# Kira7dn/Low_Level_Feature_Extraction

Hardware: AMD Instinct MI355X
Metric: images/sec, 1080p batch, full colors+shapes+shadows pipeline @1/2/4/8 MI355X (higher is better)
Workload: dtype u8

## Files before the change

### low_level_feature_extraction_amd/_build.py

```python
from __future__ import annotations

import os
import shutil
import subprocess
import sys

PKG = os.path.dirname(os.path.abspath(__file__))
ROOT = os.path.dirname(PKG)
CSRC = os.path.join(PKG, "csrc")
LIB = os.path.join(PKG, "libllfe.so")
SOURCES = ["llfe_context.cpp", "llfe_pipeline.cpp", "llfe_stages.cpp", "llfe_resize.cpp", "llfe_decode.cpp", "llfe_colors_images.cpp", "llfe_shapes_images.cpp", "contours.cpp", "png_decode.cpp", "jpeg_decode.cpp", "stencil.hip", "stencil_stream.hip", "hysteresis.hip", "unique.hip", "kmeans.hip", "kmeans_big.hip", "resize.hip", "contours_gpu.hip",
           "cvresize.hip", "text.hip", "gather.hip", "font.hip", "font_bits.hip", "jpeg_huff.hip", "png_inflate.hip", "thumb_images.hip", "jpeg_images.hip"]
HEADERS = ["llfe_ctx.h", "llfe_internal.h", "contours.h", "kmeans_common.h", "jpeg_huff_core.h", "jpeg_desc_check.h", "jpeg_recon_core.h", "jpeg_images.h", "jpeg_orient.h", "png_inflate_core.h", "host_fanout.h"]
RECOMPILE = [("kmeans.hip", "kmeans_wide", ["-DLLFE_KM_WIDE=1", "-DLLFE_KM_THREADS=512", "-DLLFE_KM_UNROLL=4"])]
ARCH = os.environ.get("LLFE_OFFLOAD_ARCH", "gfx950")
ILP_SCHED = set(filter(None, os.environ.get("LLFE_ILP_SCHED", "stencil_stream.hip,kmeans.hip").split(",")))


def _hipcc() -> str:
    for c in (os.environ.get("HIPCC"), "/opt/rocm/bin/hipcc", shutil.which("hipcc")):
        if c and os.path.exists(c):
            return c
    raise RuntimeError("hipcc not found: the llfe HIP backend cannot be built")


def _stale() -> bool:
    if not os.path.exists(LIB):
        return True
    t = os.path.getmtime(LIB)
    deps = [os.path.join(CSRC, f) for f in SOURCES + HEADERS] + [os.path.join(ROOT, "include", "llfe.h"), __file__]
    return any(os.path.getmtime(d) > t for d in deps)


def build(force: bool = False, verbose: bool = False) -> str:
    if not force and not _stale():
        return LIB
    objs = []
    hipcc = _hipcc()
    common = ["-O3", "-fPIC", "-std=c++17", "-ffp-contract=off", f"-I{os.path.join(ROOT, 'include')}",
              "-Wall", "-Wno-unused-function", "-Wno-unused-variable",
              *os.environ.get("LLFE_EXTRA_FLAGS", "").split()]
    tmpdir = os.path.join(PKG, "build")
    os.makedirs(tmpdir, exist_ok=True)
    procs = []
    for src, stem, defs in [(s, s, []) for s in SOURCES] + RECOMPILE:
        obj = os.path.join(tmpdir, stem + ".o" if stem != src else src + ".o")
        objs.append(obj)
        if src in ("contours.cpp", "png_decode.cpp", "jpeg_decode.cpp"):
            lang = ["-x", "c++"]
        else:
            lang = ["-x", "hip", f"--offload-arch={ARCH}"]
        extra = ["-fno-slp-vectorize"] if src == "stencil_stream.hip" else []
        if src in ILP_SCHED:
            extra += ["-mllvm", "-amdgpu-sched-strategy=iterative-ilp"]
        cmd = [hipcc, *common, *lang, *extra, *defs, "-c", os.path.join(CSRC, src), "-o", obj]
        if verbose:
            print(" ".join(cmd), file=sys.stderr)
        procs.append((cmd, subprocess.Popen(cmd, stdout=subprocess.PIPE, stderr=subprocess.STDOUT)))
    failed = []
    for cmd, p in procs:
        out, _ = p.communicate()
        if p.returncode != 0:
            failed.append((cmd, out.decode(errors="replace")))
        elif verbose and out:
            print(out.decode(errors="replace"), file=sys.stderr)
    if failed:
        msg = "\n\n".join(" ".join(c) + "\n" + o for c, o in failed)
        raise RuntimeError("libllfe build failed:\n" + msg)
    tmp = LIB + ".tmp"
    cmd = [hipcc, "-shared", "-fPIC", f"--offload-arch={ARCH}", *objs, "-o", tmp, "-lpthread", "-lz", "-ldl"]
    subprocess.run(cmd, check=True)
    os.replace(tmp, LIB)
    return LIB


if __name__ == "__main__":
    print(build(force="--force" in sys.argv, verbose=True))
```

### low_level_feature_extraction_amd/csrc/kmeans.hip

```cpp
#include "kmeans_common.h"

#include <mutex>
#include <type_traits>

namespace llfe {
namespace {

#ifndef LLFE_KM_CELL_MIN
#define LLFE_KM_CELL_MIN 8192
#endif
constexpr int kCellMinCubes = LLFE_KM_CELL_MIN;
#ifndef LLFE_KM_SPLIT
#define LLFE_KM_SPLIT 0
#endif
#ifndef LLFE_KM_LLOYD_QUEUE
#define LLFE_KM_LLOYD_QUEUE 0
#endif
#ifndef LLFE_KM_SUPS
#define LLFE_KM_SUPS 1
#endif
#ifndef LLFE_KM_WIDE
#define LLFE_KM_WIDE 0
#endif
#ifndef LLFE_KM_THREADS
#define LLFE_KM_THREADS 256
#endif
constexpr int KT = LLFE_KM_THREADS;
constexpr int KW = KT / 64;
constexpr int STEP = 256;
constexpr float kFar = 1e30f;

using km::cvrng_double;
using km::cvrng_next;
using km::splitmix64;

__device__ __forceinline__ float uni(float v) {
    return __int_as_float(__builtin_amdgcn_readfirstlane(__float_as_int(v)));
}

__device__ __forceinline__ float d2(float x, float y, float z, float cx, float cy, float cz) {
    float t0 = x - cx, t1 = y - cy, t2 = z - cz;
    float d = t0 * t0;
    d = __builtin_fmaf(t1, t1, d);
    d = __builtin_fmaf(t2, t2, d);
    return d;
}

struct P3 {
    float x, y, z;
};
__device__ __forceinline__ P3 unpack(uint32_t k) {
    return P3{(float)((k >> 16) & 255u), (float)((k >> 8) & 255u), (float)(k & 255u)};
}

struct Cent {
    float x[kMaxK], y[kMaxK], z[kMaxK];
};

__device__ __forceinline__ int label5(const P3 &p, const Cent &c, float &best) {
    best = d2(p.x, p.y, p.z, c.x[0], c.y[0], c.z[0]);
    int l = 0;
#pragma unroll
    for (int k = 1; k < kMaxK; k++) {
        float d = d2(p.x, p.y, p.z, c.x[k], c.y[k], c.z[k]);
        bool lt = d < best;
        best = lt ? d : best;
        l = lt ? k : l;
    }
    return l;
}

typedef float f2 __attribute__((ext_vector_type(2)));
typedef uint16_t u16x2 __attribute__((ext_vector_type(2)));
struct CentP {
    f2 x[3], y[3], z[3];
};

__device__ __forceinline__ CentP pack_centres(const Cent &c) {
    CentP r;
#pragma unroll
    for (int j = 0; j < 3; j++) {
        const int a = 2 * j, b = 2 * j + 1;
        r.x[j] = f2{c.x[a], b < kMaxK ? c.x[b] : kFar};
        r.y[j] = f2{c.y[a], b < kMaxK ? c.y[b] : kFar};
        r.z[j] = f2{c.z[a], b < kMaxK ? c.z[b] : kFar};
    }
    return r;
}

__device__ __forceinline__ int label5p(uint32_t key, const CentP &c) {
    const float x = (float)((key >> 16) & 255u), y = (float)((key >> 8) & 255u), z = (float)(key & 255u);
    const f2 px = f2{x, x}, py = f2{y, y}, pz = f2{z, z};
    f2 d[3];
#pragma unroll
    for (int j = 0; j < 3; j++) {
        const f2 t0 = px - c.x[j], t1 = py - c.y[j], t2 = pz - c.z[j];
        f2 dd = t0 * t0;
        dd = __builtin_elementwise_fma(t1, t1, dd);
        dd = __builtin_elementwise_fma(t2, t2, dd);
        d[j] = dd;
    }
    const float m = fminf(fminf(fminf(d[0].x, d[0].y), fminf(d[1].x, d[1].y)), d[2].x);
    int l = 4;
    l = d[1].y == m ? 3 : l;
    l = d[1].x == m ? 2 : l;
    l = d[0].y == m ? 1 : l;
    l = d[0].x == m ? 0 : l;
    return l;
}

constexpr int PF = 4;
constexpr int kSelSteps = ((4 * 256 * 256 + 3 + STEP - 1) / STEP + KW - 1) / KW + 1;
constexpr int SEL_U = 4;
#ifndef LLFE_KM_UNROLL
#define LLFE_KM_UNROLL 2
#endif
#ifndef LLFE_KM_SPLIT_MIN
#define LLFE_KM_SPLIT_MIN 1
#endif
constexpr bool kSplitOn = LLFE_KM_SPLIT_MIN <= 64;
constexpr int kPend = 128;
constexpr int kPendIdxBits = 18;
#ifndef LLFE_KM_PP_SPLIT_MIN
#define LLFE_KM_PP_SPLIT_MIN 8
#endif
constexpr int kPPSplitMin = LLFE_KM_PP_SPLIT_MIN;
#ifndef LLFE_KM_PPRUN
#define LLFE_KM_PPRUN 4
#endif
constexpr int kPPRun = LLFE_KM_PPRUN;
constexpr int ring_size(int need) { return need <= 256 ? 256 : (need <= 512 ? 512 : 1024); }
constexpr int kStage = ring_size(127 + 64 * LLFE_KM_UNROLL);
static_assert(kStage >= 127 + 64 * LLFE_KM_UNROLL && (kStage & (kStage - 1)) == 0, "boundary-colour ring too small");

__device__ __forceinline__ uint4 load_step(const uint32_t *pts, int s, int se_full, int lane) {
    if (s < se_full) return *(const uint4 *)(pts + (size_t)s * STEP + lane * 4);
    return make_uint4(0u, 0u, 0u, 0u);
}

template <typename T>
__device__ __forceinline__ T wave_sum(T v) {
#pragma unroll
    for (int off = 32; off > 0; off >>= 1) v += __shfl_xor(v, off);
    return v;
}

struct KmSmem {
    unsigned long long accA[kMaxK][KT];
    unsigned long long accB[kMaxK][KT];
    union {
        unsigned long long red[32][20];
        int cs[KW][256];
    };
    unsigned long long wtot[KW][3];
    unsigned long long scan_w[KW];
    double dred[KW];
    double maxd[KW];
    int maxi[KW];
    float c[kMaxK][3];
    float cprev[kMaxK][3];
    float cc[kMaxK][3];
    long long sums[kMaxK][3];
    int counts[kMaxK];
    int moved_idx[kMaxK];
    int moved_lbl[kMaxK];
    int n_moved;
    int found_step[3];
    unsigned long long found_excl[3];
    int ci[3];
    int flag;
    int task;
    int next_chunk;
    unsigned long long fail_pts;
    unsigned long long split_cubes, split_pts;
    uint32_t split_walks, split_partial;
    union {
        struct {
            unsigned long long psum[3][kParts];
            unsigned long long pD[kParts];
            unsigned long long wchunk[3][KW];
            int marg[kMaxK * kMaxK + 6 * kMaxK];
            int margc[kMaxK * kMaxK + 6 * kMaxK];
            int margs[kMaxK * kMaxK + 6 * kMaxK];
        } ppw;
        uint32_t pend[KW][kPend];
    };
    unsigned long long pex[3];
    unsigned long long S[3];
    uint32_t pbase[kParts + 1];
    uint32_t kbeg[kParts];
    uint32_t kfirst, klast;
    int pj[3];
    int icc[kMaxK][3];
    unsigned long long sel_pts;
    uint32_t stage[KW][kStage + 64];
    float thrL[3][kMaxK * kMaxK];
    int cq[KW][256];
    unsigned long long qtot;
    unsigned long long drift_hist;
};

static_assert(sizeof(KmSmem) * (1024 / KT) <= 160 * 1024, "KmSmem must leave room for 1024 / KT workgroups per CU");
static_assert(offsetof(KmSmem, accB) == sizeof(((KmSmem *)nullptr)->accA) &&
                  3 * KW * kSelSteps * sizeof(uint32_t) <= 2 * sizeof(((KmSmem *)nullptr)->accA),
              "selection step sums overflow the Lloyd accumulators (KT too small)");
static_assert(KW > 4 || sizeof(((KmSmem *)nullptr)->pend) <= sizeof(((KmSmem *)nullptr)->ppw),
              "pending-cube lists overflow the k-means++ state they alias");
static_assert(kPend >= 63 + 64 && (kPend & (kPend - 1)) == 0, "pending-cube list too small");
struct PPPend {
    uint32_t list[KW][3][kPend];
    uint32_t walks, lanes, mixed;
};
static_assert(sizeof(PPPend) % 4 == 0 && 3 * KW * kSelSteps * sizeof(uint32_t) + sizeof(PPPend) <= 2 * sizeof(((KmSmem *)nullptr)->accA),
              "k-means++ pending-cube lists overlap the selection's step sums");
__device__ __forceinline__ PPPend &pp_pend(KmSmem &sm) {
    return *reinterpret_cast<PPPend *>(reinterpret_cast<char *>(&sm.accB[0][0]) + sizeof(sm.accB) - sizeof(PPPend));
}

__device__ __forceinline__ Cent load_centres(const float (*c)[3]) {
    Cent r;
#pragma unroll
    for (int k = 0; k < kMaxK; k++) {
        r.x[k] = uni(c[k][0]);
        r.y[k] = uni(c[k][1]);
        r.z[k] = uni(c[k][2]);
    }
    return r;
}

__device__ __forceinline__ int moved_label(const KmSmem &sm, int i, int l) {
    for (int m = 0; m < sm.n_moved; m++)
        if (sm.moved_idx[m] == i) l = sm.moved_lbl[m];
    return l;
}

__device__ __forceinline__ int d2i(int x, int y, int z, int cx, int cy, int cz) {
    const int a = x - cx, b = y - cy, c = z - cz;
    return __mul24(a, a) + __mul24(b, b) + __mul24(c, c);
}

struct ICent {
    int x[kMaxK], y[kMaxK], z[kMaxK];
};

__device__ __forceinline__ bool never_closer(int ox, int oy, int oz, int ax, int ay, int az, int bx, int by, int bz) {
    const int f = d2i(ox, oy, oz, ax, ay, az) - d2i(ox, oy, oz, bx, by, bz);
    return f - 6 * (max(ax - bx, 0) + max(ay - by, 0) + max(az - bz, 0)) >= 0;
}
__device__ __forceinline__ bool always_closer(int ox, int oy, int oz, int ax, int ay, int az, int bx, int by, int bz) {
    const int f = d2i(ox, oy, oz, ax, ay, az) - d2i(ox, oy, oz, bx, by, bz);
    return f + 6 * (max(bx - ax, 0) + max(by - ay, 0) + max(bz - az, 0)) <= 0;
}

struct CubeGeo {
    int ox, oy, oz, n, sx, sy, sz, s2;
};

__device__ __forceinline__ uint32_t cube_key(uint32_t id, int bit) {
    return ((((id >> 12) & 63u) * 4u + (uint32_t)(bit >> 4)) << 16) |
           ((((id >> 6) & 63u) * 4u + (uint32_t)((bit >> 2) & 3)) << 8) | ((id & 63u) * 4u + (uint32_t)(bit & 3));
}
__device__ __forceinline__ CubeGeo cube_geo(const CubeEnt &e) {
    CubeGeo g;
    g.ox = (int)((e.id >> 12) & 63u) * 4;
    g.oy = (int)((e.id >> 6) & 63u) * 4;
    g.oz = (int)(e.id & 63u) * 4;
    g.n = (int)(e.sums & 127u);
    g.sx = (int)((e.sums >> 7) & 255u);
    g.sy = (int)((e.sums >> 15) & 255u);
    g.sz = (int)(e.sums >> 23);
    g.s2 = (int)(e.id >> 18);
    return g;
}
__device__ __forceinline__ uint32_t cube_sum(const CubeGeo &g, int cx, int cy, int cz) {
    const int ax = g.ox - cx, ay = g.oy - cy, az = g.oz - cz;
    const uint32_t q = (uint32_t)(__mul24(ax, ax) + __mul24(ay, ay) + __mul24(az, az));
    return __umul24((uint32_t)g.n, q) + 2u * (uint32_t)(__mul24(ax, g.sx) + __mul24(ay, g.sy) + __mul24(az, g.sz)) +
           (uint32_t)g.s2;
}

__device__ __forceinline__ uint32_t lane_sel(unsigned long long m, uint32_t a, uint32_t b) {
    uint32_t r;
    asm("v_cndmask_b32_e64 %0, %2, %1, %3" : "=v"(r) : "v"(a), "v"(b), "s"(m));
    return r;
}

__device__ __forceinline__ unsigned long long clear_bit(unsigned long long m, int b) {
    asm("s_bitset0_b64 %0, %1" : "+s"(m) : "s"(b));
    return m;
}

__device__ __forceinline__ uint32_t lane_offset(int lane) {
    return ((uint32_t)(lane >> 4) << 16) | ((uint32_t)((lane >> 2) & 3) << 8) | (uint32_t)(lane & 3);
}
__device__ __forceinline__ uint32_t cube_origin_key(uint32_t id) {
    return ((((id >> 12) & 63u) * 4u) << 16) | ((((id >> 6) & 63u) * 4u) << 8) | ((id & 63u) * 4u);
}

constexpr int kBisFrac = 10;
constexpr int kBisBand = 1 << (kBisFrac - 1);

__device__ __forceinline__ uint4 bisector_signs(int p, int s1, int s2, int s3) {
    int n = 2 * kBisBand - p;
    uint32_t w[4] = {0u, 0u, 0u, 0u};
#pragma unroll
    for (int bit = 63; bit >= 0; bit--) {
        const int h = bit >> 5;
        w[h] = __builtin_amdgcn_alignbit(w[h], (uint32_t)p, 31);
        w[2 + h] = __builtin_amdgcn_alignbit(w[2 + h], (uint32_t)n, 31);
        if (bit > 0) {
            const int s = (bit & 15) == 0 ? s3 : ((bit & 3) == 0 ? s2 : s1);
            p += s;
            n -= s;
        }
    }
    return make_uint4(w[0], w[1], w[2], w[3]);
}

struct MaskMoments {
    uint32_t n, sx, sy, sz;
};
__device__ __forceinline__ MaskMoments mask_moments(uint32_t lo, uint32_t hi) {
    MaskMoments r;
    const uint32_t nh = __popc(hi);
    r.n = __popc(lo) + nh;
    r.sx = __popc(lo & 0xFFFF0000u) + __popc(hi & 0xFFFF0000u) + 2u * nh;
    r.sy = __popc(lo & 0xF0F0F0F0u) + __popc(hi & 0xF0F0F0F0u) + 2u * (__popc(lo & 0xFF00FF00u) + __popc(hi & 0xFF00FF00u));
    r.sz = __popc(lo & 0xAAAAAAAAu) + __popc(hi & 0xAAAAAAAAu) + 2u * (__popc(lo & 0xCCCCCCCCu) + __popc(hi & 0xCCCCCCCCu));
    return r;
}

__device__ __forceinline__ uint4 split_drain(KmSmem &sm, const CubeEnt *__restrict__ ctab, const uint32_t *pl, int first, int n) {
    const int tid = threadIdx.x, lane = tid & 63;
    uint4 r = make_uint4(0u, 0u, 0u, 0u);
    if (lane < n) {
        const uint32_t ent = pl[(first + lane) & (kPend - 1)];
        const CubeEnt e = ctab[ent & ((1u << kPendIdxBits) - 1u)];
        const int k = (int)((ent >> kPendIdxBits) & 7u), jc = (int)(ent >> (kPendIdxBits + 3));
        const int ox = (int)((e.id >> 12) & 63u) * 4, oy = (int)((e.id >> 6) & 63u) * 4, oz = (int)(e.id & 63u) * 4;
        int p, s1, s2, s3;
        {
            const float *ck = sm.c[k], *cj = sm.c[jc];
            const float ax = ck[0] - cj[0], ay = ck[1] - cj[1], az = ck[2] - cj[2];
            const float bx = (float)(2 * ox) - (cj[0] + ck[0]), by = (float)(2 * oy) - (cj[1] + ck[1]),
                        bz = (float)(2 * oz) - (cj[2] + ck[2]);
            const float f0 = __builtin_fmaf(az, bz, __builtin_fmaf(ay, by, ax * bx));
            constexpr float sc = (float)(1 << kBisFrac);
            const int gx = (int)__builtin_rintf(ax * (2.f * sc)), gy = (int)__builtin_rintf(ay * (2.f * sc)),
                      gz = (int)__builtin_rintf(az * (2.f * sc));
            p = kBisBand - ((int)__builtin_rintf(f0 * sc) + 3 * (gx + gy + gz));
            s1 = gz;
            s2 = gy - 3 * gz;
            s3 = gx - 3 * (gy + gz);
        }
        const uint32_t mlo = (uint32_t)e.mask, mhi = (uint32_t)(e.mask >> 32);
        const uint4 sg = bisector_signs(p, s1, s2, s3);
        const MaskMoments a = mask_moments(mlo & sg.x, mhi & sg.y), b = mask_moments(mlo & sg.z, mhi & sg.w);
        atomicAdd(&sm.accA[k][tid], (unsigned long long)(a.n * (uint32_t)ox + a.sx) |
                                        ((unsigned long long)(a.n * (uint32_t)oy + a.sy) << 32));
        atomicAdd(&sm.accB[k][tid], (unsigned long long)(a.n * (uint32_t)oz + a.sz) | ((unsigned long long)a.n << 32));
        atomicAdd(&sm.accA[jc][tid], (unsigned long long)(b.n * (uint32_t)ox + b.sx) |
                                         ((unsigned long long)(b.n * (uint32_t)oy + b.sy) << 32));
        atomicAdd(&sm.accB[jc][tid], (unsigned long long)(b.n * (uint32_t)oz + b.sz) | ((unsigned long long)b.n << 32));
        r.x = mlo & ~(sg.x | sg.z);
        r.y = mhi & ~(sg.y | sg.w);
        r.z = cube_origin_key(e.id);
        r.w = a.n + b.n;
    }
    return r;
}

__device__ __forceinline__ uint2 gain_signs(int q, int s1, int s2, int s3) {
    uint32_t w[2] = {0u, 0u};
#pragma unroll
    for (int bit = 63; bit >= 0; bit--) {
        const int h = bit >> 5;
        w[h] = __builtin_amdgcn_alignbit(w[h], (uint32_t)q, 31);
        if (bit > 0) q += (bit & 15) == 0 ? s3 : ((bit & 3) == 0 ? s2 : s1);
    }
    return make_uint2(w[0], w[1]);
}

__device__ __forceinline__ uint32_t pp_walk(KmSmem &sm, int first, int n, int head, uint32_t tk0, uint32_t tk1, uint32_t tk2) {
    const int lane = threadIdx.x & 63, wid = threadIdx.x >> 6;
    uint32_t(*pl)[kPend] = pp_pend(sm).list[wid];
    uint32_t rest = 0u, mlo = 0u, mhi = 0u, ent = 0u;
    int R = -1;
    if (lane < n) {
        const uint32_t slot = (uint32_t)(first + lane) & (kPend - 1);
        mlo = pl[0][slot];
        mhi = pl[1][slot];
        ent = pl[2][slot];
        const int k = (int)(ent >> (kPendIdxBits + 3));
        const uint32_t und = (ent >> kPendIdxBits) & 7u;
        const int j = __builtin_ctz(und);
        rest = und & (und - 1u);
        R = (int)((ent >> 12) & 63u);
        const int ox = R * 4, oy = (int)((ent >> 6) & 63u) * 4, oz = (int)(ent & 63u) * 4;
        const int kx = sm.icc[k][0], ky = sm.icc[k][1], kz = sm.icc[k][2];
        const uint32_t tk = j == 0 ? tk0 : (j == 1 ? tk1 : tk2);
        const int tjx = (int)(tk >> 16), tjy = (int)((tk >> 8) & 255u), tjz = (int)(tk & 255u);
        const int f = d2i(ox, oy, oz, tjx, tjy, tjz) - d2i(ox, oy, oz, kx, ky, kz);
        const int gx = 2 * (tjx - kx), gy = 2 * (tjy - ky), gz = 2 * (tjz - kz);
        const uint2 pos = gain_signs(f - 3 * (gx + gy + gz), gz, gy - 3 * gz, gx - 3 * (gy + gz));
        const MaskMoments a = mask_moments(mlo & pos.x, mhi & pos.y);
        const uint32_t g = (uint32_t)(__mul24(gx, (int)a.sx) + __mul24(gy, (int)a.sy) + __mul24(gz, (int)a.sz) - __mul24((int)a.n, f));
        if (g) atomicAdd(&(&sm.ppw.psum[0][0])[j * kParts + R], (unsigned long long)g);
    }
    const unsigned long long rb = __ballot(rest != 0u);
    if (rest) {
        const uint32_t slot = ((uint32_t)head + __builtin_amdgcn_mbcnt_hi((uint32_t)(rb >> 32), __builtin_amdgcn_mbcnt_lo((uint32_t)rb, 0u))) & (kPend - 1);
        pl[0][slot] = mlo;
        pl[1][slot] = mhi;
        pl[2][slot] = (ent & ~(7u << kPendIdxBits)) | (rest << kPendIdxBits);
    }
    const uint32_t mixed = __ballot(lane < n && R != __builtin_amdgcn_readfirstlane(R)) != 0ull;
    return (uint32_t)__popcll(rb) | (mixed << 7);
}

struct PPSplit {
    uint32_t und;
    int k;
};

__device__ __forceinline__ uint32_t lane_off_rel(int fill) { return (uint32_t)(__lane_id() - fill); }

constexpr int CPF = 1;
struct CubeRing {
    CubeEnt r[CPF];
    __device__ __forceinline__ void init(const CubeEnt *t, int cb, int cend, int lane) {
#pragma unroll
        for (int q = 0; q < CPF; q++) {
            r[q].mask = 0;
            r[q].id = 0;
            r[q].sums = 0;
            if (cb + q * 64 + lane < cend) r[q] = t[cb + q * 64 + lane];
        }
    }
    __device__ __forceinline__ CubeEnt next(const CubeEnt *t, int ci, int cend) {
        const CubeEnt e = r[0];
#pragma unroll
        for (int q = 0; q + 1 < CPF; q++) r[q] = r[q + 1];
        if (ci + CPF * 64 < cend) r[CPF - 1] = t[ci + CPF * 64];
        return e;
    }
};
// ... 1003 lines not shown
                l2 += ok ? v2 : 0u;
            }
            uint32_t a0 = wave_sum(l0), a1 = wave_sum(l1), a2 = wave_sum(l2);
            if (lane == 0) {
                o0[s] = a0;
                o1[s] = a1;
                o2[s] = a2;
            }
            wt0 += a0;
            wt1 += a1;
            wt2 += a2;
        }
        if (lane == 0) {
            sm.wtot[wid][0] = wt0;
            sm.wtot[wid][1] = wt1;
            sm.wtot[wid][2] = wt2;
        }
        __syncthreads();
        unsigned long long S[3] = {0, 0, 0};
        for (int w = 0; w < KW; w++)
            for (int j = 0; j < 3; j++) S[j] += sm.wtot[w][j];
        int best = 0;
        double bs = 1.7976931348623157e308;
        for (int j = 0; j < 3; j++)
            if ((double)S[j] < bs) {
                bs = (double)S[j];
                best = j;
            }
        sum0 = S[best];
        cur = best == 0 ? sl0 : (best == 1 ? sl1 : sl2);
        __syncthreads();
        if (tid == 0) {
            sm.cc[kk][0] = tc.x[best];
            sm.cc[kk][1] = tc.y[best];
            sm.cc[kk][2] = tc.z[best];
        }
        __syncthreads();
    }

    }
    if (tid == 0) o->t_pp = wall_clock64();
    if (tid < kMaxK * 3) (&o->pp_centers[0][0])[tid] = sm.cc[tid / 3][tid % 3];
    }
    if (kPhase == 1) {
        if (tid < kMaxK * 3) (&o->centers[0][0])[(tid / 3) * 3 + tid % 3] = sm.cc[tid / 3][tid % 3];
        if (tid == 0) {
            o->qtot = sm.qtot;
            o->bytes = bytes;
            o->pp_pts = pp_pts;
            o->pp_split_cubes = pp_split_cubes;
            o->pp_split_pts = pp_split_pts;
            o->pp_walks = pp_walks.x;
            o->pp_walk_lanes = pp_walks.y;
            o->pp_walk_mixed = pp_walks.z;
            o->pad = (int32_t)pp_sel;
            o->t_sel = t_sel;
        }
        goto next_task;
    }
    if (kPhase == 2) {
        if (tid < kMaxK * 3) {
            const int k = tid / 3, j = tid % 3;
            sm.cc[k][j] = k < K ? o->centers[k][j] : kFar;
        }
        if (tid == 0) sm.qtot = o->qtot;
        bytes = o->bytes;
        __syncthreads();
    }
    if (tid < kMaxK * 3) {
        int k = tid / 3, j = tid % 3;
        sm.c[k][j] = k < K ? sm.cc[k][j] : kFar;
    }
    __syncthreads();

    auto thr_tables = [&](int q) {
        const int k = q / kMaxK, j = q % kMaxK;
        const float dx = fabsf(sm.c[j][0] - sm.c[k][0]), dy = fabsf(sm.c[j][1] - sm.c[k][1]),
                    dz = fabsf(sm.c[j][2] - sm.c[k][2]);
        const bool none = j == k || j >= K || k >= K;
        sm.thrL[0][q] = none ? -__builtin_inff() : 3.f * (dx + dy + dz) + 1.f;
        sm.thrL[1][q] = none ? -__builtin_inff() : 3.f * dx + 7.f * (dy + dz) + 1.f;
        sm.thrL[2][q] = none ? -__builtin_inff() : 3.f * dx + 15.f * (dy + dz) + 1.f;
    };
    if (tid == 0) sm.next_chunk = 0;
    if (use_cubes && tid < kMaxK * kMaxK) thr_tables(tid);
#pragma unroll
    for (int k = 0; k < kMaxK; k++) {
        sm.accA[k][tid] = 0;
        sm.accB[k][tid] = 0;
    }
    __syncthreads();
    int iter = 1;
    const double eps2 = 0.2 * 0.2;
    uint64_t t_sw = 0;
    if (tid == 0) sm.drift_hist = 0;
    for (;;) {
        const uint64_t tsw0 = wall_clock64();
        const CentP c = pack_centres(load_centres(sm.c));
        if (use_cubes) {
            const Cent cu = load_centres(sm.c);
            f2 lw_x[3], lw_y[3], lw_z[3], lc2[3];
#pragma unroll
            for (int j = 0; j < 3; j++) {
#pragma unroll
                for (int h = 0; h < 2; h++) {
                    const int m = 2 * j + h;
                    const bool used = m < K;
                    const float cx = m < kMaxK ? cu.x[m] : 0.f, cy = m < kMaxK ? cu.y[m] : 0.f,
                                cz = m < kMaxK ? cu.z[m] : 0.f;
                    const float wx = used ? -2.f * cx : 0.f, wy = used ? -2.f * cy : 0.f, wz = used ? -2.f * cz : 0.f;
                    const float c2 = used ? cx * cx + cy * cy + cz * cz : __builtin_inff();
                    if (h == 0) {
                        lw_x[j].x = wx, lw_y[j].x = wy, lw_z[j].x = wz, lc2[j].x = c2;
                    } else {
                        lw_x[j].y = wx, lw_y[j].y = wy, lw_z[j].y = wz, lc2[j].y = c2;
                    }
                }
            }
            unsigned long long fails = 0;
            uint32_t *stg = sm.stage[wid];
            const uint32_t loff = lane_offset(lane);
            int head = 0, tail = 0;
            uint32_t spl = 0;
            auto label_stage = [&](int count) {
                __builtin_amdgcn_wave_barrier();
                if (lane < count) {
                    const uint32_t kq = stg[(tail + lane) & (kStage - 1)];
                    const int l = label5p(kq, c);
                    atomicAdd(&sm.accA[l][tid], (unsigned long long)((kq >> 16) & 255u) |
                                                    ((unsigned long long)((kq >> 8) & 255u) << 32));
                    atomicAdd(&sm.accB[l][tid], (unsigned long long)(kq & 255u) | (1ull << 32));
                }
                tail += count;
            };
            auto label_stage2 = [&]() {
                __builtin_amdgcn_wave_barrier();
                const uint32_t k0 = stg[(tail + lane) & (kStage - 1)], k1 = stg[(tail + 64 + lane) & (kStage - 1)];
                const int l0 = label5p(k0, c), l1 = label5p(k1, c);
                atomicAdd(&sm.accA[l0][tid], (unsigned long long)((k0 >> 16) & 255u) |
                                                 ((unsigned long long)((k0 >> 8) & 255u) << 32));
                atomicAdd(&sm.accB[l0][tid], (unsigned long long)(k0 & 255u) | (1ull << 32));
                atomicAdd(&sm.accA[l1][tid], (unsigned long long)((k1 >> 16) & 255u) |
                                                 ((unsigned long long)((k1 >> 8) & 255u) << 32));
                atomicAdd(&sm.accB[l1][tid], (unsigned long long)(k1 & 255u) | (1ull << 32));
                tail += 128;
            };
#define LABEL_FULL() while (head - tail >= 128) label_stage2()
            auto grab = [&]() {
                int b = 0;
                if (lane == 0) b = atomicAdd(&sm.next_chunk, 64);
                return b;
            };
            auto push_cubes = [&](unsigned long long fm, const uint32_t mlo, const uint32_t mhi,
                                  const uint32_t okey) __attribute__((always_inline)) {
                auto push = [&](int src) {
                    const unsigned long long m =
                        ((unsigned long long)(uint32_t)__builtin_amdgcn_readlane(mhi, src) << 32) |
                        (uint32_t)__builtin_amdgcn_readlane(mlo, src);
                    const uint32_t k = __builtin_amdgcn_readlane(okey, src);
                    const uint32_t r =
                        __builtin_amdgcn_mbcnt_hi((uint32_t)(m >> 32), __builtin_amdgcn_mbcnt_lo((uint32_t)m, 0u));
                    stg[lane_sel(m, ((uint32_t)head + r) & (kStage - 1), kStage + lane)] = k | loff;
                    head += __popcll(m);
                };
                while (fm) {
#pragma unroll
                    for (int u = 0; u < LLFE_KM_UNROLL; u++) {
                        if (u > 0 && !fm) break;
// ... 361 lines not shown

        for (int ek = 0; ek < K; ek++) {
            if (sm.counts[ek] != 0) continue;
            int max_k = 0;
            for (int k1 = 1; k1 < K; k1++)
                if (sm.counts[max_k] < sm.counts[k1]) max_k = k1;
            const float scale = 1.f / (float)sm.counts[max_k];
            const float bx = (float)sm.sums[max_k][0] * scale, by = (float)sm.sums[max_k][1] * scale,
                        bz = (float)sm.sums[max_k][2] * scale;
            const Cent cp = load_centres(sm.cprev);
            double md = -1.0;
            int mi = -1;
            auto visit = [&](int i) {
                P3 pp = unpack(pts[i]);
                float bd;
                int l = moved_label(sm, i, label5(pp, cp, bd));
                if (l != max_k) return;
                double d = (double)d2(pp.x, pp.y, pp.z, bx, by, bz);
                if (md <= d) {
                    md = d;
                    mi = i;
                }
            };
            if (kCubes && cubes.part_hist) {
                if (wid == 0) (void)key_layout(sm, cubes.part_uq + (size_t)img * kParts,
                                               cubes.part_hist + (size_t)img * kParts, 0u);
                __syncthreads();
                for (int P = 0; P < kParts; P++) {
                    const int a0 = (int)sm.kbeg[P], a1 = a0 + (int)(sm.pbase[P + 1] - sm.pbase[P]);
                    for (int i = a0 + tid; i < a1; i += KT) visit(i);
                }
            } else {
                for (int s = sb; s < se; s++) {
                    const int i0 = s * STEP + lane * 4;
                    for (int jj = 0; jj < 4; jj++) {
                        const int i = i0 + jj;
                        if (i >= N) break;
                        visit(i);
                    }
                }
            }
#pragma unroll
            for (int off = 32; off > 0; off >>= 1) {
                double od = __shfl_xor(md, off);
                int oi = __shfl_xor(mi, off);
                if (od > md || (od == md && oi > mi)) {
                    md = od;
                    mi = oi;
                }
            }
            if (lane == 0) {
                sm.maxd[wid] = md;
                sm.maxi[wid] = mi;
            }
            __syncthreads();
            if (tid == 0) {
                double bd2 = -1.0;
                int bi = -1;
                for (int w = 0; w < KW; w++)
                    if (sm.maxd[w] > bd2 || (sm.maxd[w] == bd2 && sm.maxi[w] > bi)) {
                        bd2 = sm.maxd[w];
                        bi = sm.maxi[w];
                    }
                if (bi >= 0) {
                    P3 pp = unpack(pts[bi]);
                    sm.counts[max_k]--;
                    sm.counts[ek]++;
                    sm.sums[max_k][0] -= (long long)pp.x;
                    sm.sums[max_k][1] -= (long long)pp.y;
                    sm.sums[max_k][2] -= (long long)pp.z;
                    sm.sums[ek][0] += (long long)pp.x;
                    sm.sums[ek][1] += (long long)pp.y;
                    sm.sums[ek][2] += (long long)pp.z;
                    sm.moved_idx[sm.n_moved] = bi;
                    sm.moved_lbl[sm.n_moved] = ek;
                    sm.n_moved++;
                }
            }
            __syncthreads();
        }
        }
        iter++;
        if (sm.flag) break;
    }

    if (tid == 0) {
        o->t_lloyd = wall_clock64();
        bytes += (unsigned long long)(iter - 1) * (use_cubes ? 16ull * (unsigned long long)C : 4ull * (unsigned long long)N);
        ll_pts = sm.fail_pts;
    }
    if (use_cubes) {
        if (tid == 0) {
            double acc = (double)sm.qtot;
            for (int k = 0; k < K; k++) {
                double cs = 0.0, c2 = 0.0;
                for (int j = 0; j < 3; j++) {
                    const double cj = (double)sm.c[k][j];
                    cs += cj * (double)sm.sums[k][j];
                    c2 += cj * cj;
                }
                acc -= 2.0 * cs - (double)sm.counts[k] * c2;
            }
            sm.dred[0] = acc;
            for (int w = 1; w < KW; w++) sm.dred[w] = 0.0;
        }
        __syncthreads();
    } else {
        const Cent cp = load_centres(sm.cprev);
        const Cent cn = load_centres(sm.c);
        const bool moved = sm.n_moved > 0;
        double acc = 0.0;
        for (int s = sb; s < se; s++) {
            const int i0 = s * STEP + lane * 4;
            for (int jj = 0; jj < 4; jj++) {
                const int i = i0 + jj;
                if (i >= N) break;
                P3 pp = unpack(pts[i]);
                float bd;
                int l = label5(pp, cp, bd);
                if (moved) l = moved_label(sm, i, l);
                float cx = cn.x[0], cy = cn.y[0], cz = cn.z[0];
#pragma unroll
                for (int k = 1; k < kMaxK; k++) {
                    cx = l == k ? cn.x[k] : cx;
                    cy = l == k ? cn.y[k] : cy;
                    cz = l == k ? cn.z[k] : cz;
                }
                acc += (double)d2(pp.x, pp.y, pp.z, cx, cy, cz);
            }
        }
        acc = wave_sum(acc);
        if (lane == 0) sm.dred[wid] = acc;
        __syncthreads();
    }
    {
        if (tid == 0) {
            double compactness = 0.0;
            for (int w = 0; w < KW; w++) compactness += sm.dred[w];
            o->compactness = compactness;
            o->iters = iter;
            o->bytes = bytes;
            if (kPhase & 1) {
                o->pp_pts = pp_pts;
                o->pp_split_cubes = pp_split_cubes;
                o->pp_split_pts = pp_split_pts;
                o->pp_walks = pp_walks.x;
                o->pp_walk_lanes = pp_walks.y;
                o->pp_walk_mixed = pp_walks.z;
                o->pad = (int32_t)pp_sel;
                o->t_sel = t_sel;
            }
            o->ll_pts = ll_pts;
            o->split_cubes = sm.split_cubes;
            o->split_pts = sm.split_pts;
            o->split_walks = sm.split_walks;
            o->split_partial = sm.split_partial;
            o->t_sw = t_sw;
            o->n_cubes = (uint32_t)C;
            o->drift_hist = sm.drift_hist;
            o->t_end = wall_clock64();
            for (int k = 0; k < kMaxK; k++) {
                for (int j = 0; j < 3; j++) o->centers[k][j] = k < K ? sm.c[k][j] : 0.f;
                o->counts[k] = k < K ? sm.counts[k] : 0;
            }
        }
    }
// ... 173 lines not shown
```

Measured before the change: 38390.

## Classify boundary cubes via per-pair sorted lattice tables instead of bit-serial sign sweep

For the non-wide k-means kernel, precomputes per centre-pair tables in shared memory (sorted lattice values and cumulative masks), rebuilt each Lloyd iteration. Boundary cubes are then classified with rank lookups and a short walk rather than the 64-step bisector sign sweep. The aim is to cut per-cube ALU work in the cube-assignment path. The cost is extra shared memory, a table rebuild plus a barrier per iteration, and data-dependent loops that can diverge across lanes.

```diff
diff --git a/low_level_feature_extraction_amd/_build.py b/low_level_feature_extraction_amd/_build.py
--- a/low_level_feature_extraction_amd/_build.py
+++ b/low_level_feature_extraction_amd/_build.py
@@ -11,7 +11,7 @@
 LIB = os.path.join(PKG, "libllfe.so")
 SOURCES = ["llfe_context.cpp", "llfe_pipeline.cpp", "llfe_stages.cpp", "llfe_resize.cpp", "llfe_decode.cpp", "llfe_colors_images.cpp", "llfe_shapes_images.cpp", "contours.cpp", "png_decode.cpp", "jpeg_decode.cpp", "stencil.hip", "stencil_stream.hip", "hysteresis.hip", "unique.hip", "kmeans.hip", "kmeans_big.hip", "resize.hip", "contours_gpu.hip",
            "cvresize.hip", "text.hip", "gather.hip", "font.hip", "font_bits.hip", "jpeg_huff.hip", "png_inflate.hip", "thumb_images.hip", "jpeg_images.hip"]
-HEADERS = ["llfe_ctx.h", "llfe_internal.h", "contours.h", "kmeans_common.h", "jpeg_huff_core.h", "jpeg_desc_check.h", "jpeg_recon_core.h", "jpeg_images.h", "jpeg_orient.h", "png_inflate_core.h", "host_fanout.h"]
+HEADERS = ["llfe_ctx.h", "llfe_internal.h", "contours.h", "kmeans_common.h", "kmeans_lattice.h", "jpeg_huff_core.h", "jpeg_desc_check.h", "jpeg_recon_core.h", "jpeg_images.h", "jpeg_orient.h", "png_inflate_core.h", "host_fanout.h"]
 RECOMPILE = [("kmeans.hip", "kmeans_wide", ["-DLLFE_KM_WIDE=1", "-DLLFE_KM_THREADS=512", "-DLLFE_KM_UNROLL=4"])]
 ARCH = os.environ.get("LLFE_OFFLOAD_ARCH", "gfx950")
 ILP_SCHED = set(filter(None, os.environ.get("LLFE_ILP_SCHED", "stencil_stream.hip,kmeans.hip").split(",")))
diff --git a/low_level_feature_extraction_amd/csrc/kmeans.hip b/low_level_feature_extraction_amd/csrc/kmeans.hip
--- a/low_level_feature_extraction_amd/csrc/kmeans.hip
+++ b/low_level_feature_extraction_amd/csrc/kmeans.hip
@@ -2,6 +2,8 @@
 
 #include <mutex>
 #include <type_traits>
+
+#include "kmeans_lattice.h"
 
 namespace llfe {
 namespace {
@@ -119,6 +121,11 @@
 #define LLFE_KM_SPLIT_MIN 1
 #endif
 constexpr bool kSplitOn = LLFE_KM_SPLIT_MIN <= 64;
+constexpr bool kLattice = !LLFE_KM_WIDE;
+constexpr int kPairs = kMaxK * (kMaxK - 1) / 2;
+static_assert(kMaxK == 5, "llfe_kml::pair_index numbers the pairs of five centres");
+static_assert(!kLattice || 16 * kPairs <= KT, "one thread per position of every pair table");
+static_assert(llfe_kml::kFrac == 10, "kmeans_lattice.h and the band analysis below share the fixed point");
 constexpr int kPend = 128;
 constexpr int kPendIdxBits = 18;
 #ifndef LLFE_KM_PP_SPLIT_MIN
@@ -198,6 +205,9 @@
     int cq[KW][256];
     unsigned long long qtot;
     unsigned long long drift_hist;
+#if !LLFE_KM_WIDE
+    llfe_kml::PairTable pair[kPairs];
+#endif
 };
 
 static_assert(sizeof(KmSmem) * (1024 / KT) <= 160 * 1024, "KmSmem must leave room for 1024 / KT workgroups per CU");
@@ -338,30 +348,36 @@
         const CubeEnt e = ctab[ent & ((1u << kPendIdxBits) - 1u)];
         const int k = (int)((ent >> kPendIdxBits) & 7u), jc = (int)(ent >> (kPendIdxBits + 3));
         const int ox = (int)((e.id >> 12) & 63u) * 4, oy = (int)((e.id >> 6) & 63u) * 4, oz = (int)(e.id & 63u) * 4;
-        int p, s1, s2, s3;
+        const float *ck = sm.c[k], *cj = sm.c[jc];
+        const float ax = ck[0] - cj[0], ay = ck[1] - cj[1], az = ck[2] - cj[2];
+        const float bx = (float)(2 * ox) - (cj[0] + ck[0]), by = (float)(2 * oy) - (cj[1] + ck[1]),
+                    bz = (float)(2 * oz) - (cj[2] + ck[2]);
+        const float f0 = __builtin_fmaf(az, bz, __builtin_fmaf(ay, by, ax * bx));
+        constexpr float sc = (float)(1 << kBisFrac);
+        const int f0q = (int)__builtin_rintf(f0 * sc);
+        const uint32_t mlo = (uint32_t)e.mask, mhi = (uint32_t)(e.mask >> 32);
+        uint4 sg;
+        int ka = k, kb = jc;
+#if !LLFE_KM_WIDE
         {
-            const float *ck = sm.c[k], *cj = sm.c[jc];
-            const float ax = ck[0] - cj[0], ay = ck[1] - cj[1], az = ck[2] - cj[2];
-            const float bx = (float)(2 * ox) - (cj[0] + ck[0]), by = (float)(2 * oy) - (cj[1] + ck[1]),
-                        bz = (float)(2 * oz) - (cj[2] + ck[2]);
-            const float f0 = __builtin_fmaf(az, bz, __builtin_fmaf(ay, by, ax * bx));
-            constexpr float sc = (float)(1 << kBisFrac);
+            ka = min(k, jc), kb = max(k, jc);
+            const llfe_kml::Sides sd = llfe_kml::lattice_sides(f0q, sm.pair[llfe_kml::pair_index(ka, kb)], k > jc);
+            sg = make_uint4(sd.lo_x, sd.lo_y, sd.hi_x, sd.hi_y);
+        }
+#else
+        {
             const int gx = (int)__builtin_rintf(ax * (2.f * sc)), gy = (int)__builtin_rintf(ay * (2.f * sc)),
                       gz = (int)__builtin_rintf(az * (2.f * sc));
-            p = kBisBand - ((int)__builtin_rintf(f0 * sc) + 3 * (gx + gy + gz));
-            s1 = gz;
-            s2 = gy - 3 * gz;
-            s3 = gx - 3 * (gy + gz);
-        }
-        const uint32_t mlo = (uint32_t)e.mask, mhi = (uint32_t)(e.mask >> 32);
-        const uint4 sg = bisector_signs(p, s1, s2, s3);
+            sg = bisector_signs(kBisBand - (f0q + 3 * (gx + gy + gz)), gz, gy - 3 * gz, gx - 3 * (gy + gz));
+        }
+#endif
         const MaskMoments a = mask_moments(mlo & sg.x, mhi & sg.y), b = mask_moments(mlo & sg.z, mhi & sg.w);
-        atomicAdd(&sm.accA[k][tid], (unsigned long long)(a.n * (uint32_t)ox + a.sx) |
-                                        ((unsigned long long)(a.n * (uint32_t)oy + a.sy) << 32));
-        atomicAdd(&sm.accB[k][tid], (unsigned long long)(a.n * (uint32_t)oz + a.sz) | ((unsigned long long)a.n << 32));
-        atomicAdd(&sm.accA[jc][tid], (unsigned long long)(b.n * (uint32_t)ox + b.sx) |
+        atomicAdd(&sm.accA[ka][tid], (unsigned long long)(a.n * (uint32_t)ox + a.sx) |
+                                         ((unsigned long long)(a.n * (uint32_t)oy + a.sy) << 32));
+        atomicAdd(&sm.accB[ka][tid], (unsigned long long)(a.n * (uint32_t)oz + a.sz) | ((unsigned long long)a.n << 32));
+        atomicAdd(&sm.accA[kb][tid], (unsigned long long)(b.n * (uint32_t)ox + b.sx) |
                                          ((unsigned long long)(b.n * (uint32_t)oy + b.sy) << 32));
-        atomicAdd(&sm.accB[jc][tid], (unsigned long long)(b.n * (uint32_t)oz + b.sz) | ((unsigned long long)b.n << 32));
+        atomicAdd(&sm.accB[kb][tid], (unsigned long long)(b.n * (uint32_t)oz + b.sz) | ((unsigned long long)b.n << 32));
         r.x = mlo & ~(sg.x | sg.z);
         r.y = mhi & ~(sg.y | sg.w);
         r.z = cube_origin_key(e.id);
@@ -1531,8 +1547,27 @@
         sm.thrL[1][q] = none ? -__builtin_inff() : 3.f * dx + 7.f * (dy + dz) + 1.f;
         sm.thrL[2][q] = none ? -__builtin_inff() : 3.f * dx + 15.f * (dy + dz) + 1.f;
     };
+    const bool lattice = kLattice && use_cubes && C >= kCellMinCubes;
+    auto pair_tables = [&](int t) {
+#if !LLFE_KM_WIDE
+        const int p = t >> 4, q = t & 15;
+        const int lo = llfe_kml::pair_lo(p), hi = llfe_kml::pair_hi(p);
+        if (p < kPairs && hi < K) {
+            llfe_kml::PairTable &pt = sm.pair[p];
+            const int gx = llfe_kml::lattice_step(sm.c[lo][0], sm.c[hi][0]), gy = llfe_kml::lattice_step(sm.c[lo][1], sm.c[hi][1]),
+                      gz = llfe_kml::lattice_step(sm.c[lo][2], sm.c[hi][2]);
+            llfe_kml::lattice_place(pt, q, gx, gy, gz);
+            __builtin_amdgcn_wave_barrier();
+            uint32_t x = pt.mm[q + 1];
+#pragma unroll
+            for (int d = 1; d < 16; d <<= 1) x |= (uint32_t)__shfl_down((int)x, d, 16);
+            pt.mm[q + 1] = (uint16_t)x;
+        }
+#endif
+    };
     if (tid == 0) sm.next_chunk = 0;
     if (use_cubes && tid < kMaxK * kMaxK) thr_tables(tid);
+    if (lattice) pair_tables(tid);
 #pragma unroll
     for (int k = 0; k < kMaxK; k++) {
         sm.accA[k][tid] = 0;
@@ -2060,6 +2095,10 @@
         }
         iter++;
         if (sm.flag) break;
+        if (lattice) {
+            pair_tables(tid);
+            __syncthreads();
+        }
     }
 
     if (tid == 0) {
diff --git a/low_level_feature_extraction_amd/csrc/kmeans_lattice.h b/low_level_feature_extraction_amd/csrc/kmeans_lattice.h
--- /dev/null
+++ b/low_level_feature_extraction_amd/csrc/kmeans_lattice.h
@@ -0,0 +1,169 @@
+#ifndef LLFE_KMEANS_LATTICE_H
+#define LLFE_KMEANS_LATTICE_H
+#include <cstddef>
+#include <cstdint>
+
+#if defined(__HIPCC__)
+#include <hip/hip_runtime.h>
+#define LLFE_KML_HD __host__ __device__ __forceinline__
+#else
+#define LLFE_KML_HD inline
+#endif
+
+namespace llfe_kml {
+
+constexpr int kFrac = 10;
+constexpr int kBand = 1 << (kFrac - 1);
+
+struct alignas(16) PairTable {
+    int32_t c[4];
+    int32_t gxy[2];
+    int32_t vb[18];
+    int32_t gz;
+    uint16_t mm[18];
+    uint32_t pad[2];
+};
+static_assert(sizeof(PairTable) == 144, "PairTable layout");
+
+LLFE_KML_HD int pair_index(int lo, int hi) { return ((lo * (9 - lo)) >> 1) + hi - lo - 1; }
+LLFE_KML_HD int pair_lo(int p) { return (p >= 4) + (p >= 7) + (p >= 9); }
+LLFE_KML_HD int pair_hi(int p) {
+    const int lo = pair_lo(p);
+    return p - ((lo * (9 - lo)) >> 1) + lo + 1;
+}
+
+LLFE_KML_HD int lattice_step(float c_lo, float c_hi) {
+    return (int)__builtin_rintf((c_lo - c_hi) * (2.f * (float)(1 << kFrac)));
+}
+LLFE_KML_HD int lattice_value(int q, int gy, int gz) { return gy * (q >> 2) + gz * (q & 3); }
+LLFE_KML_HD int lattice_rank(int q, int gy, int gz) {
+    const int v = lattice_value(q, gy, gz);
+    int r = 0;
+#if defined(__HIP_DEVICE_COMPILE__)
+#pragma unroll
+#endif
+    for (int o = 0; o < 16; o++) {
+        const int w = lattice_value(o, gy, gz);
+        r += (w < v) | ((w == v) & (o < q));
+    }
+    return r;
+}
+
+LLFE_KML_HD void lattice_place(PairTable &t, int q, int gx, int gy, int gz) {
+    const int v = lattice_value(q, gy, gz), r = lattice_rank(q, gy, gz);
+    t.vb[r + 2] = v;
+    if ((r & 3) == 3) t.c[r >> 2] = v;
+    t.mm[r + 1] = (uint16_t)(1u << q);
+    if (q == 0) {
+        t.gxy[0] = gx, t.gxy[1] = gy, t.gz = gz;
+        t.vb[0] = t.vb[1] = INT32_MIN;
+        t.mm[0] = 0xFFFF, t.mm[17] = 0;
+    }
+}
+
+LLFE_KML_HD void lattice_build(const float c_lo[3], const float c_hi[3], PairTable &t) {
+    const int gx = lattice_step(c_lo[0], c_hi[0]), gy = lattice_step(c_lo[1], c_hi[1]), gz = lattice_step(c_lo[2], c_hi[2]);
+    for (int q = 0; q < 16; q++) lattice_place(t, q, gx, gy, gz);
+    for (int r = 14; r >= 0; r--) t.mm[r + 1] = (uint16_t)(t.mm[r + 1] | t.mm[r + 2]);
+    t.pad[0] = t.pad[1] = 0u;
+}
+
+LLFE_KML_HD int count_le(int n, int v, int a) {
+#if defined(__HIP_DEVICE_COMPILE__)
+    asm("v_cmp_le_i32 vcc, %1, %2\n\tv_addc_co_u32 %0, vcc, 0, %0, vcc" : "+v"(n) : "v"(v), "v"(a) : "vcc");
+    return n;
+#else
+    return n + (v <= a);
+#endif
+}
+
+struct __attribute__((aligned(16), may_alias)) Quad {
+    int32_t x, y, z, w;
+};
+static_assert(offsetof(PairTable, c) % 16 == 0 && offsetof(PairTable, vb) % 16 == 8, "the 16-byte reads of PairTable");
+
+LLFE_KML_HD void lattice_ranks(const PairTable &t, const int a[4], int r[4]) {
+    const Quad c = *reinterpret_cast<const Quad *>(&t.c[0]);
+    int h[4];
+#if defined(__HIP_DEVICE_COMPILE__)
+#pragma unroll
+#endif
+    for (int s = 0; s < 4; s++) {
+        const int n = count_le(count_le(count_le(count_le(0, c.x, a[s]), c.y, a[s]), c.z, a[s]), c.w, a[s]);
+        h[s] = n < 3 ? n : 3;
+    }
+#if defined(__HIP_DEVICE_COMPILE__)
+#pragma unroll
+#endif
+    for (int s = 0; s < 4; s++) {
+        const Quad b = reinterpret_cast<const Quad *>(&t.vb[2])[h[s]];
+        r[s] = count_le(count_le(count_le(count_le(4 * h[s], b.x, a[s]), b.y, a[s]), b.z, a[s]), b.w, a[s]);
+    }
+}
+
+struct Sides {
+    uint32_t lo_x, lo_y, hi_x, hi_y;
+};
+LLFE_KML_HD Sides lattice_sides(int f0q, const PairTable &t, bool owner_hi) {
+    const int gx = t.gxy[0];
+    const int a0 = kBand + (owner_hi ? f0q : -f0q);
+    int a[4], b[4], ra[4];
+#if defined(__HIP_DEVICE_COMPILE__)
+#pragma unroll
+#endif
+    for (int s = 0; s < 4; s++) {
+        a[s] = a0 - gx * s;
+        b[s] = a[s] - (2 * kBand + 1);
+    }
+    lattice_ranks(t, a, ra);
+    uint32_t ma[4], mb[4];
+    int rb[4], pv[4];
+    bool deep[4];
+#if defined(__HIP_DEVICE_COMPILE__)
+#pragma unroll
+#endif
+    for (int s = 0; s < 4; s++) {
+        const int p2 = t.vb[ra[s]], p1 = t.vb[ra[s] + 1];
+        const uint32_t m1 = t.mm[ra[s]], m0 = t.mm[ra[s] + 1];
+        ma[s] = m0;
+        mb[s] = p1 > b[s] ? m1 : m0;
+        rb[s] = ra[s] - 1;
+        pv[s] = p2;
+        deep[s] = p2 > b[s];
+    }
+    if (deep[0] | deep[1] | deep[2] | deep[3]) {
+        do {
+#if defined(__HIP_DEVICE_COMPILE__)
+#pragma unroll
+#endif
+            for (int s = 0; s < 4; s++) {
+                if (pv[s] > b[s]) {
+                    rb[s]--;
+                    pv[s] = t.vb[rb[s] + 1];
+                }
+            }
+        } while ((pv[0] > b[0]) | (pv[1] > b[1]) | (pv[2] > b[2]) | (pv[3] > b[3]));
+#if defined(__HIP_DEVICE_COMPILE__)
+#pragma unroll
+#endif
+        for (int s = 0; s < 4; s++)
+            if (deep[s]) mb[s] = t.mm[rb[s] + 1];
+    }
+    Sides o;
+    o.lo_x = ma[0] | (ma[1] << 16);
+    o.lo_y = ma[2] | (ma[3] << 16);
+    o.hi_x = ~(mb[0] | (mb[1] << 16));
+    o.hi_y = ~(mb[2] | (mb[3] << 16));
+    return o;
+}
+
+struct Signs {
+    uint32_t x, y, z, w;
+};
+LLFE_KML_HD Signs lattice_signs(int f0q, const PairTable &t, bool owner_hi) {
+    const Sides s = lattice_sides(f0q, t, owner_hi);
+    return owner_hi ? Signs{s.hi_x, s.hi_y, s.lo_x, s.lo_y} : Signs{s.lo_x, s.lo_y, s.hi_x, s.hi_y};
+}
+
+}
+#endif
```

Result: faster. 39210, median of 6 (+2.1%).
